# cure-lab/MagicDrive

Measured on NVIDIA B200. Metric: 6-view 224x400 denoising-steps/sec, higher is better.
Workload: dtype bf16

## Files before the change

magicdrive_b200/csrc/attention_tc.cuh:

```cuda
#pragma once
#include "ptx.cuh"

namespace mdb {

constexpr int ATT_BM = 128;
constexpr int ATT_BN = 128;

constexpr int ATT_MAX_SRC = 3;
struct AttnKvMaps {
  CUtensorMap k[ATT_MAX_SRC], v[ATT_MAX_SRC];
};

struct AttnTcParams {
  __nv_bfloat16* out;
  int ldo;
  int lq, lk;
  const int* kv_index;
  int n_sets;
  int n_src;
  float scale_log2;
  int q_step;
  long long* trace;
};

template <int D>
struct AttnTcCfg {
  static constexpr int KD = (D + 63) / 64;
  static constexpr int D16 = (D + 15) / 16 * 16;
  static constexpr int STAGES = (D <= 80) ? 2 : 1;
  static constexpr int TILE = ATT_BM * 128;
  static constexpr int SMEM_Q = KD * TILE;
  static constexpr int SMEM_KV = STAGES * 2 * KD * TILE;
  static constexpr int kSmemBytes = SMEM_Q + SMEM_KV + 1024 + 128 + 2 * 2 * ATT_BM * 4 ;
  static constexpr int S_COL = 0;
  static constexpr int P_COL = ATT_BN;
  static constexpr int O_COL = ATT_BN + 64;
  static constexpr int kTmemCols = (ATT_BN + 64 + D16 <= 256) ? 256 : 512;
  static constexpr int HW = D16 / 2;
  static constexpr int kThreads = 64 + 8 * 32;
};

__device__ __forceinline__ void umma_bf16_ts(uint32_t tmem_d, uint32_t tmem_a, uint64_t bdesc, uint32_t idesc,
                                             uint32_t accumulate) {
  asm volatile(
      "{\n\t"
      ".reg .pred p;\n\t"
      "setp.ne.b32 p, %4, 0;\n\t"
      "tcgen05.mma.cta_group::1.kind::f16 [%0], [%1], %2, %3, p;\n\t"
      "}\n" ::"r"(tmem_d),
      "r"(tmem_a), "l"(bdesc), "r"(idesc), "r"(accumulate)
      : "memory");
}

__device__ __forceinline__ void tmem_st_32x16(uint32_t taddr, const uint32_t (&v)[16]) {
  asm volatile(
      "tcgen05.st.sync.aligned.32x32b.x16.b32 [%0], "
      "{%1, %2, %3, %4, %5, %6, %7, %8, %9, %10, %11, %12, %13, %14, %15, %16};" ::"r"(taddr),
      "r"(v[0]), "r"(v[1]), "r"(v[2]), "r"(v[3]), "r"(v[4]), "r"(v[5]), "r"(v[6]), "r"(v[7]), "r"(v[8]), "r"(v[9]),
      "r"(v[10]), "r"(v[11]), "r"(v[12]), "r"(v[13]), "r"(v[14]), "r"(v[15])
      : "memory");
}
__device__ __forceinline__ void tmem_st_32x8(uint32_t taddr, const uint32_t (&v)[8]) {
  asm volatile("tcgen05.st.sync.aligned.32x32b.x8.b32 [%0], {%1, %2, %3, %4, %5, %6, %7, %8};" ::"r"(taddr), "r"(v[0]),
               "r"(v[1]), "r"(v[2]), "r"(v[3]), "r"(v[4]), "r"(v[5]), "r"(v[6]), "r"(v[7])
               : "memory");
}
__device__ __forceinline__ void tmem_st_wait() { asm volatile("tcgen05.wait::st.sync.aligned;" ::: "memory"); }

__device__ __forceinline__ uint64_t make_sw128_mnmajor_desc(uint32_t smem_addr_bytes, uint32_t lbo_bytes) {
  uint64_t d = 0;
  d |= static_cast<uint64_t>((smem_addr_bytes >> 4) & 0x3FFF);
  d |= static_cast<uint64_t>((lbo_bytes >> 4) & 0x3FFF) << 16;
  d |= static_cast<uint64_t>((1024u >> 4) & 0x3FFF) << 32;
  d |= static_cast<uint64_t>(1) << 46;
  d |= static_cast<uint64_t>(2) << 61;
  return d;
}

template <int D>
__global__ void __launch_bounds__(AttnTcCfg<D>::kThreads, (D <= 64) ? 2 : 1)
attention_tc_kernel(const __grid_constant__ CUtensorMap tmQ, const __grid_constant__ AttnKvMaps kvm,
                    const AttnTcParams p) {
  using Cfg = AttnTcCfg<D>;
  constexpr int KD = Cfg::KD, D16 = Cfg::D16, STAGES = Cfg::STAGES, TILE = Cfg::TILE;
  extern __shared__ uint8_t smem_raw[];
  uint8_t* smem = reinterpret_cast<uint8_t*>((reinterpret_cast<uintptr_t>(smem_raw) + 1023) & ~uintptr_t(1023));
  uint8_t* smQ = smem;
  uint8_t* smK = smQ + Cfg::SMEM_Q;
  uint8_t* smV = smK + STAGES * KD * TILE;
  uint64_t* bars = reinterpret_cast<uint64_t*>(smV + STAGES * KD * TILE);
  uint64_t* q_full = bars;
  uint64_t* kv_full = bars + 1;
  uint64_t* kv_empty = bars + 3;
  uint64_t* s_full = bars + 5;
  uint64_t* p_full = bars + 6;
  uint64_t* o_full = bars + 7;
  uint64_t* o_free = bars + 8;
  uint32_t* tmem_slot = reinterpret_cast<uint32_t*>(bars + 9);
  float* xchg = reinterpret_cast<float*>(bars + 16);

  const int warp = threadIdx.x >> 5, lane = threadIdx.x & 31;
  const int b = blockIdx.z, head = blockIdx.y, q0 = blockIdx.x * ATT_BM;
  const int ntiles = (p.lk + ATT_BN - 1) / ATT_BN;
  const int total_iters = ntiles * p.n_sets;

  if (warp == 0 && lane == 0) {
    prefetch_tmap(&tmQ);
    for (int i = 0; i < p.n_src; ++i) {
      prefetch_tmap(&kvm.k[i]);
      prefetch_tmap(&kvm.v[i]);
    }
  }
  if (warp == 1 && lane == 0) {
    mbar_init(q_full, 1);
    for (int i = 0; i < 2; ++i) {
      mbar_init(&kv_full[i], 1);
      mbar_init(&kv_empty[i], 1);
    }
    mbar_init(s_full, 1);
    mbar_init(p_full, 8);
    mbar_init(o_full, 1);
    mbar_init(o_free, 8);
    fence_barrier_init();
  }
  if (warp == 2) {
    tmem_alloc(tmem_slot, Cfg::kTmemCols);
    tmem_relinquish();
  }
  tc_fence_before();
  __syncthreads();
  tc_fence_after();
  const uint32_t tmem_base = *tmem_slot;
  asm volatile("griddepcontrol.wait;" ::: "memory");
  asm volatile("griddepcontrol.launch_dependents;" ::: "memory");

  if (warp == 0) {
    if (elect_one()) {
      mbar_arrive_expect_tx(q_full, KD * TILE);
#pragma unroll
      for (int c = 0; c < KD; ++c) tma_load_4d(&tmQ, q_full, smQ + c * TILE, c * 64, head, q0, b);
      int stage = 0;
      uint32_t phase = 0;
      for (int set = 0; set < p.n_sets; ++set) {
        const int kve = p.kv_index ? p.kv_index[b * p.n_sets + set] : b;
        const int kvb = kve & 0xffffff;
        const CUtensorMap* km = &kvm.k[kve >> 24];
        const CUtensorMap* vm = &kvm.v[kve >> 24];
        for (int j = 0; j < ntiles; ++j) {
          mbar_wait(&kv_empty[stage], phase ^ 1);
          mbar_arrive_expect_tx(&kv_full[stage], 2 * KD * TILE);
#pragma unroll
          for (int c = 0; c < KD; ++c) {
            tma_load_4d(km, &kv_full[stage], smK + (stage * KD + c) * TILE, c * 64, head, j * ATT_BN, kvb);
            tma_load_4d(vm, &kv_full[stage], smV + (stage * KD + c) * TILE, c * 64, head, j * ATT_BN, kvb);
          }
          if (++stage == STAGES) {
            stage = 0;
            phase ^= 1;
          }
        }
      }
    }
  } else if (warp == 1) {
    constexpr uint32_t idesc_s = make_idesc_bf16(ATT_BM, ATT_BN);
    constexpr uint32_t idesc_o = make_idesc_bf16(ATT_BM, D16) | (1u << 16);
    const uint32_t tmem_s = tmem_base + Cfg::S_COL;
    const uint32_t tmem_o = tmem_base + Cfg::O_COL;
    mbar_wait(q_full, 0);
    int stage = 0;
    uint32_t phase = 0;
    auto issue_s = [&](int st) {
      if (elect_one()) {
#pragma unroll
        for (int k = 0; k < D16 / 16; ++k) {
          const int c = k / 4, kk = k % 4;
          const uint64_t adesc = make_sw128_kmajor_desc(smem_u32(smQ + c * TILE)) + 2 * kk;
          const uint64_t bdesc = make_sw128_kmajor_desc(smem_u32(smK + (st * KD + c) * TILE)) + 2 * kk;
          umma_bf16(tmem_s, adesc, bdesc, idesc_s, k > 0 ? 1u : 0u);
        }
        umma_commit(s_full);
      }
      __syncwarp();
    };
    mbar_wait(&kv_full[0], 0);
    tc_fence_after();
    issue_s(0);
    for (int it = 0; it < total_iters; ++it) {
      mbar_wait(p_full, it & 1);
      mbar_wait(o_free, (it & 1) ^ 1);
      tc_fence_after();
      if (elect_one()) {
#pragma unroll
        for (int k = 0; k < ATT_BN / 16; ++k) {
          const uint64_t bdesc = make_sw128_mnmajor_desc(smem_u32(smV + stage * KD * TILE), TILE) + (2048u >> 4) * k;
          umma_bf16_ts(tmem_o, tmem_base + Cfg::P_COL + 8 * k, bdesc, idesc_o, k > 0 ? 1u : 0u);
        }
        umma_commit(o_full);
        umma_commit(&kv_empty[stage]);
      }
      __syncwarp();
      if (++stage == STAGES) {
        stage = 0;
        phase ^= 1;
      }
      if (it + 1 < total_iters) {
        mbar_wait(&kv_full[stage], phase);
        tc_fence_after();
        issue_s(stage);
      }
    }
  } else {
    constexpr int HW = Cfg::HW;
    const int q = warp & 3;
    const int hlf = (warp - 2) >> 2;
    const int row = q * 32 + lane;
    const uint32_t lane_base = tmem_base + (static_cast<uint32_t>(q * 32) << 16);
    const uint32_t tmem_s = lane_base + Cfg::S_COL + hlf * 64;
    const uint32_t tmem_p = lane_base + Cfg::P_COL + hlf * 32;
    const uint32_t tmem_o = lane_base + Cfg::O_COL + hlf * HW;
    const int qrow = q0 + row;
    __nv_bfloat16* orow = p.out + (static_cast<long long>(b) * p.lq + qrow) * p.ldo + head * D + hlf * HW;
    constexpr int NVALID = (D - HW >= HW) ? HW : (D - HW);
    const int nvalid = hlf ? NVALID : HW;
    const float sc = p.scale_log2;
    int it = 0;
    for (int set = 0; set < p.n_sets; ++set) {
      float o[HW];
#pragma unroll
      for (int i = 0; i < HW; ++i) o[i] = 0.f;
      float m = -INFINITY, l = 0.f;
      for (int j = 0; j < ntiles; ++j, ++it) {
        mbar_wait(s_full, it & 1);
        tc_fence_after();
        const int kbase = j * ATT_BN + hlf * 64;
        const bool tail = (kbase + 64 > p.lk);
        float mx = -INFINITY;
#pragma unroll 1
        for (int c = 0; c < 64; c += 32) {
          uint32_t v[32];
          tmem_ld_32x32(tmem_s + c, v);
          tmem_ld_wait();
          if (!tail) {
#pragma unroll
            for (int i = 0; i < 32; ++i) mx = fmaxf(mx, __uint_as_float(v[i]));
          } else {
#pragma unroll
            for (int i = 0; i < 32; ++i)
              if (kbase + c + i < p.lk) mx = fmaxf(mx, __uint_as_float(v[i]));
          }
        }
        float* xb = xchg + (it & 1) * 256;
        xb[hlf * 128 + row] = mx;
        asm volatile("bar.sync %0, 64;" ::"r"(1 + q) : "memory");
        mx = fmaxf(mx, xb[(hlf ^ 1) * 128 + row]);
        const float m_new = fmaxf(m, mx * sc);
        const float corr = exp2f(m - m_new);
        m = m_new;
        float rs = 0.f;
#pragma unroll 1
        for (int c = 0; c < 64; c += 32) {
          uint32_t v[32];
          tmem_ld_32x32(tmem_s + c, v);
          tmem_ld_wait();
          uint32_t pk[16];
          if (!tail) {
#pragma unroll
            for (int i = 0; i < 32; i += 2) {
              const float p0 = exp2f(fmaf(__uint_as_float(v[i]), sc, -m_new));
              const float p1 = exp2f(fmaf(__uint_as_float(v[i + 1]), sc, -m_new));
              rs += p0 + p1;
              pk[i >> 1] = pack_bf16(p0, p1);
            }
          } else {
#pragma unroll
            for (int i = 0; i < 32; i += 2) {
              const float p0 = (kbase + c + i < p.lk) ? exp2f(fmaf(__uint_as_float(v[i]), sc, -m_new)) : 0.f;
              const float p1 = (kbase + c + i + 1 < p.lk) ? exp2f(fmaf(__uint_as_float(v[i + 1]), sc, -m_new)) : 0.f;
              rs += p0 + p1;
              pk[i >> 1] = pack_bf16(p0, p1);
            }
          }
          tmem_st_32x16(tmem_p + (c >> 1), pk);
        }
        tmem_st_wait();
        l = l * corr + rs;
        tc_fence_before();
        __syncwarp();
        if (lane == 0) mbar_arrive(p_full);
        mbar_wait(o_full, it & 1);
        tc_fence_after();
#pragma unroll
        for (int c = 0; c < HW; c += 8) {
          uint32_t v[8];
          tmem_ld_32x8(tmem_o + c, v);
          tmem_ld_wait();
#pragma unroll
          for (int i = 0; i < 8; ++i) o[c + i] = o[c + i] * corr + __uint_as_float(v[i]);
        }
        tc_fence_before();
        __syncwarp();
        if (lane == 0) mbar_arrive(o_free);
      }
      float* xb = xchg + (it & 1) * 256;
      asm volatile("bar.sync %0, 64;" ::"r"(1 + q) : "memory");
      xb[hlf * 128 + row] = l;
      asm volatile("bar.sync %0, 64;" ::"r"(1 + q) : "memory");
      const float inv = 1.0f / (l + xb[(hlf ^ 1) * 128 + row]);
      asm volatile("bar.sync %0, 64;" ::"r"(1 + q) : "memory");
      if (qrow < p.lq) {
#pragma unroll
        for (int c = 0; c < HW; c += 8) {
          if (c >= nvalid) break;
          float f[8];
#pragma unroll
          for (int i = 0; i < 8; ++i) f[i] = o[c + i] * inv;
          if (set > 0) {
            const uint4 prev = *reinterpret_cast<const uint4*>(orow + c);
            const __nv_bfloat162* ph = reinterpret_cast<const __nv_bfloat162*>(&prev);
#pragma unroll
            for (int i = 0; i < 4; ++i) {
              const float2 pf = __bfloat1622float2(ph[i]);
              f[2 * i] = __bfloat162float(__float2bfloat16_rn(f[2 * i])) + pf.x;
              f[2 * i + 1] = __bfloat162float(__float2bfloat16_rn(f[2 * i + 1])) + pf.y;
            }
          }
          *reinterpret_cast<uint4*>(orow + c) =
              make_uint4(pack_bf16(f[0], f[1]), pack_bf16(f[2], f[3]), pack_bf16(f[4], f[5]), pack_bf16(f[6], f[7]));
        }
      }
    }
  }

  __syncthreads();
  if (warp == 2) {
    tc_fence_after();
    tmem_dealloc(tmem_base, Cfg::kTmemCols);
  }
}

}
```

magicdrive_b200/csrc/capi_attention.cu:

```cuda
#include <cuda_bf16.h>
#include <cuda_runtime.h>

#include <stdlib.h>

#include "../../include/magicdrive_b200.h"
#define MDB_NEED_TENSORMAP
#include "common_host.h"
#include <string.h>
#include "attention_tc.cuh"
#include "attention_tc2.cuh"

static long long* g_attn_trace = nullptr;

namespace {

bool make_qkv_map(CUtensorMap* m, const void* ptr, int d, int heads, int l, int b, int ld) {
  mdb::EncodeTiledFn enc = mdb::get_encode();
  if (!enc) return false;
  cuuint64_t dims[4] = {(cuuint64_t)d, (cuuint64_t)heads, (cuuint64_t)l, (cuuint64_t)b};
  cuuint64_t strides[3] = {(cuuint64_t)d * 2, (cuuint64_t)ld * 2, (cuuint64_t)l * ld * 2};
  cuuint32_t box[4] = {64u, 1u, (cuuint32_t)mdb::ATT_BM, 1u};
  cuuint32_t estr[4] = {1u, 1u, 1u, 1u};
  return enc(m, CU_TENSOR_MAP_DATA_TYPE_BFLOAT16, 4, const_cast<void*>(ptr), dims, strides, box, estr,
             CU_TENSOR_MAP_INTERLEAVE_NONE, CU_TENSOR_MAP_SWIZZLE_128B, CU_TENSOR_MAP_L2_PROMOTION_L2_256B,
             CU_TENSOR_MAP_FLOAT_OOB_FILL_NONE) == CUDA_SUCCESS;
}

struct KvSources {
  const void* k[mdb::ATT_MAX_SRC];
  const void* v[mdb::ATT_MAX_SRC];
  int ldk[mdb::ATT_MAX_SRC], ldv[mdb::ATT_MAX_SRC], b_kv[mdb::ATT_MAX_SRC];
  int n;
};

bool make_kv_maps(mdb::AttnKvMaps* m, const KvSources& s, int d, int heads, int lk) {
  for (int i = 0; i < mdb::ATT_MAX_SRC; ++i) {
    const int j = i < s.n ? i : 0;
    if (!make_qkv_map(&m->k[i], s.k[j], d, heads, lk, s.b_kv[j], s.ldk[j]) ||
        !make_qkv_map(&m->v[i], s.v[j], d, heads, lk, s.b_kv[j], s.ldv[j]))
      return false;
  }
  return true;
}

int attn_num_sms() {
  static int sms = 0;
  if (!sms) {
    int dev = 0;
    cudaGetDevice(&dev);
    if (cudaDeviceGetAttribute(&sms, cudaDevAttrMultiProcessorCount, dev) != cudaSuccess || sms <= 0) sms = 148;
  }
  return sms;
}

int multi_q_step(int b, int heads, int lq, int lk, int n_sets) {
  if (lk > mdb::ATT_BN || n_sets != 1) return 0;
  const char* e = getenv("MDB_ATTN_MULTIQ");
  if (e && e[0] == '0') return 0;
  const int nq = (lq + mdb::ATT_BM - 1) / mdb::ATT_BM;
  const long long per_tile_ctas = static_cast<long long>(b) * heads;
  const long long slots = 2LL * attn_num_sms();
  if (per_tile_ctas * nq <= slots) return 0;
  long long gx = slots / per_tile_ctas;
  if (gx < 1) gx = 1;
  if (gx >= nq) return 0;
  return static_cast<int>(gx);
}

template <typename Cfg, typename Kernel>
int launch_tc(Kernel kernel, const char* name, const void* q, int ldq, const KvSources& src, void* out, int ldo, int b, int heads,
              int lq, int lk, int d, const int* kv_index, int n_sets, float scale, cudaStream_t st, bool* attr, bool allow_multi_q = false) {
  if (!*attr) {
    cudaError_t e = cudaFuncSetAttribute(kernel, cudaFuncAttributeMaxDynamicSharedMemorySize, Cfg::kSmemBytes);
    if (e != cudaSuccess) return mdb::set_error(MDB_ERR_CUDA, "%s smem attr: %s", name, cudaGetErrorString(e));
    *attr = true;
  }
  CUtensorMap tq;
  mdb::AttnKvMaps kvm;
  if (!make_qkv_map(&tq, q, d, heads, lq, b, ldq) || !make_kv_maps(&kvm, src, d, heads, lk))
    return mdb::set_error(MDB_ERR_CUDA, "mdb_attention: cuTensorMapEncodeTiled failed (d=%d heads=%d lq=%d lk=%d)", d, heads, lq, lk);
  mdb::AttnTcParams p;
  p.out = static_cast<__nv_bfloat16*>(out);
  p.ldo = ldo, p.lq = lq, p.lk = lk, p.kv_index = kv_index, p.n_sets = n_sets, p.n_src = src.n;
  p.scale_log2 = scale * 1.4426950408889634f;
  p.trace = g_attn_trace;
  p.q_step = allow_multi_q ? multi_q_step(b, heads, lq, lk, n_sets) : 0;
  dim3 grid(p.q_step > 0 ? p.q_step : (lq + mdb::ATT_BM - 1) / mdb::ATT_BM, heads, b);
  cudaError_t le = mdb::launch_pdl(kernel, grid, dim3(Cfg::kThreads), Cfg::kSmemBytes, st, tq, kvm, p);
  if (le != cudaSuccess) return mdb::set_error(MDB_ERR_CUDA, "%s launch: %s", name, cudaGetErrorString(le));
  cudaError_t e2 = cudaGetLastError();
  if (e2 != cudaSuccess) return mdb::set_error(MDB_ERR_CUDA, "%s: %s", name, cudaGetErrorString(e2));
  return MDB_OK;
}

template <int D>
int launch_attention_tc(const void* q, int ldq, const KvSources& src, void* out, int ldo, int b, int heads, int lq, int lk,
                        const int* kv_index, int n_sets, float scale, cudaStream_t st) {
  static bool attr = false;
  return launch_tc<mdb::AttnTcCfg<D>>(mdb::attention_tc_kernel<D>, "attention_tc_kernel", q, ldq, src, out, ldo, b, heads, lq, lk, D,
                                      kv_index, n_sets, scale, st, &attr);
}

template <int D, bool DOUBLE_S>
int launch_attention_tc2(const void* q, int ldq, const KvSources& src, void* out, int ldo, int b, int heads, int lq, int lk,
                         const int* kv_index, int n_sets, float scale, cudaStream_t st) {
  if constexpr (!DOUBLE_S) {
    if (multi_q_step(b, heads, lq, lk, n_sets) > 0) {
      static bool attr_mq = false;
      return launch_tc<mdb::AttnTc2Cfg<D, false>>(mdb::attention_tc2_kernel<D, false, true>, "attention_tc2_kernel<multi-Q>", q, ldq, src,
                                                  out, ldo, b, heads, lq, lk, D, kv_index, n_sets, scale, st, &attr_mq, true);
    }
  }
  static bool attr = false;
  return launch_tc<mdb::AttnTc2Cfg<D, DOUBLE_S>>(mdb::attention_tc2_kernel<D, DOUBLE_S, false>, "attention_tc2_kernel", q, ldq, src, out,
                                                 ldo, b, heads, lq, lk, D, kv_index, n_sets, scale, st, &attr, false);
}

enum class AttnKernel { kTc, kTc2, kTc2Double };
AttnKernel attention_kernel_choice() {
  const char* e = getenv("MDB_ATTN_KERNEL");
  if (e && !strcmp(e, "tc2d")) return AttnKernel::kTc2Double;
  if (e && !strcmp(e, "tc")) return AttnKernel::kTc;
  return AttnKernel::kTc2;
}

int attention_dispatch(const void* q, int ldq, const KvSources& src, void* out, int ldo, int b, int heads, int lq, int lk, int d,
                       const int* kv_index, int n_sets, float scale, cudaStream_t st) {
  using namespace mdb;
  const AttnKernel which = attention_kernel_choice();
#define MDB_TC2(DD, DBL) return launch_attention_tc2<DD, DBL>(q, ldq, src, out, ldo, b, heads, lq, lk, kv_index, n_sets, scale, st)
  if (which != AttnKernel::kTc) {
    const bool dbl = which == AttnKernel::kTc2Double;
    switch (d) {
      case 40: if (dbl) MDB_TC2(40, true); else MDB_TC2(40, false);
      case 32: if (dbl) MDB_TC2(32, true); else MDB_TC2(32, false);
      case 64: if (dbl) MDB_TC2(64, true); else MDB_TC2(64, false);
      case 80: MDB_TC2(80, true);
      default: break;
    }
  }
#undef MDB_TC2
  switch (d) {
    case 40: return launch_attention_tc<40>(q, ldq, src, out, ldo, b, heads, lq, lk, kv_index, n_sets, scale, st);
    case 80: return launch_attention_tc<80>(q, ldq, src, out, ldo, b, heads, lq, lk, kv_index, n_sets, scale, st);
    case 160: return launch_attention_tc<160>(q, ldq, src, out, ldo, b, heads, lq, lk, kv_index, n_sets, scale, st);
    case 32: return launch_attention_tc<32>(q, ldq, src, out, ldo, b, heads, lq, lk, kv_index, n_sets, scale, st);
    case 64: return launch_attention_tc<64>(q, ldq, src, out, ldo, b, heads, lq, lk, kv_index, n_sets, scale, st);
    default: return set_error(MDB_ERR_UNSUPPORTED, "mdb_attention: head dim %d not instantiated (32, 40, 64, 80, 160)", d);
  }
}

}

extern "C" int mdb_attention_multi(const void* q, int ldq, int n_src, const void* const* k, const int* ldk, const void* const* v,
                                   const int* ldv, const int* b_kv, void* out, int ldo, int b, int heads, int lq, int lk, int d,
                                   const int* kv_index, int n_sets, float scale, void* stream) {
  using namespace mdb;
  if (!q || !k || !v || !ldk || !ldv || !b_kv || !out) return set_error(MDB_ERR_INVALID, "mdb_attention: null pointer");
  if (n_src < 1 || n_src > ATT_MAX_SRC) return set_error(MDB_ERR_INVALID, "mdb_attention: 1..%d K/V sources", ATT_MAX_SRC);
  if (n_sets < 1 || n_sets > 2 || (n_sets == 2 && !kv_index))
    return set_error(MDB_ERR_INVALID, "mdb_attention: n_sets must be 1 or 2 (2 needs kv_index)");
  if (scale <= 0.f) return set_error(MDB_ERR_INVALID, "mdb_attention: scale must be positive");
  if (lq <= 0 || lk <= 0 || b <= 0 || heads <= 0) return set_error(MDB_ERR_INVALID, "mdb_attention: bad shape");
  if (ldq % 8 || ldo % 8) return set_error(MDB_ERR_UNSUPPORTED, "mdb_attention: strides must be multiples of 8");
  KvSources src;
  src.n = n_src;
  for (int i = 0; i < n_src; ++i) {
    if (!k[i] || !v[i] || b_kv[i] <= 0) return set_error(MDB_ERR_INVALID, "mdb_attention: bad K/V source %d", i);
    if (ldk[i] % 8 || ldv[i] % 8) return set_error(MDB_ERR_UNSUPPORTED, "mdb_attention: strides must be multiples of 8");
    src.k[i] = k[i], src.v[i] = v[i], src.ldk[i] = ldk[i], src.ldv[i] = ldv[i], src.b_kv[i] = b_kv[i];
  }
  if (!kv_index && (n_src != 1 || b_kv[0] != b)) return set_error(MDB_ERR_INVALID, "mdb_attention: b_kv != b or several sources need kv_index");
  return attention_dispatch(q, ldq, src, out, ldo, b, heads, lq, lk, d, kv_index, n_sets, scale, static_cast<cudaStream_t>(stream));
}

extern "C" int mdb_attention(const void* q, int ldq, const void* k, int ldk, const void* v, int ldv, void* out, int ldo, int b,
                             int b_kv, int heads, int lq, int lk, int d, const int* kv_index, int n_sets, float scale,
                             void* stream) {
  return mdb_attention_multi(q, ldq, 1, &k, &ldk, &v, &ldv, &b_kv, out, ldo, b, heads, lq, lk, d, kv_index, n_sets, scale, stream);
}

extern "C" int mdb_attention_debug_trace(void* device_i64_384) {
  g_attn_trace = static_cast<long long*>(device_i64_384);
  return MDB_OK;
}
```

Measured before the change: 122.7.

## Add persistent ping-pong attention kernel processing two Q tiles per CTA

Adds a persistent attention kernel in which each CTA owns pairs of 128-row Q tiles. Two softmax warpgroups alternate, so the tensor-core QK/PV work for one tile overlaps the softmax of the other, and a 4-stage K/V TMA pipeline is shared between them. The kernel becomes the default for long Q sequences with head dim 32/40/64 and more than one K tile. The aim is to hide softmax latency and remove per-tile launch and setup cost, in exchange for a complex barrier protocol, full TMEM use and heavy shared-memory use that limit occupancy to one CTA per SM.

```diff
diff --git a/magicdrive_b200/csrc/attention_pp.cuh b/magicdrive_b200/csrc/attention_pp.cuh
--- /dev/null
+++ b/magicdrive_b200/csrc/attention_pp.cuh
@@ -0,0 +1,436 @@
+#pragma once
+#include "attention_tc2.cuh"
+
+namespace mdb {
+
+template <int D>
+struct AttnPpCfg {
+  static constexpr int KD = (D + 63) / 64;
+  static constexpr int D16 = (D + 15) / 16 * 16;
+  static constexpr int TILE = ATT_BM * 128;
+  static constexpr int STAGES = 4;
+  static constexpr int SMEM_Q = 2 * 2 * KD * TILE;
+  static constexpr int SMEM_KV = STAGES * 2 * KD * TILE;
+  static constexpr int kSmemBytes = SMEM_Q + SMEM_KV + 1024  + 256  + 2 * 2 * 2 * ATT_BM * 4 ;
+  static constexpr int kTmemCols = 512;
+  static constexpr int HW = D16 / 2;
+  static constexpr int kThreads = 64 + 16 * 32;
+  __host__ __device__ static constexpr int o_col(int t, int half) { return 256 + t * 128 + half * 64; }
+  static_assert(KD == 1 && D16 <= 64, "two O accumulators per tile at 64-column spacing");
+  static_assert(kSmemBytes <= 227 * 1024, "shared memory");
+};
+
+constexpr int ATT_PP_BAR_AB = 9, ATT_PP_BAR_BA = 10;
+
+template <int D>
+__global__ void __launch_bounds__(AttnPpCfg<D>::kThreads, 1)
+attention_pp_kernel(const __grid_constant__ CUtensorMap tmQ, const __grid_constant__ AttnKvMaps kvm, const AttnTcParams p) {
+  using Cfg = AttnPpCfg<D>;
+  constexpr int KD = Cfg::KD, D16 = Cfg::D16, STAGES = Cfg::STAGES, TILE = Cfg::TILE, HW = Cfg::HW;
+  extern __shared__ uint8_t smem_raw[];
+  uint8_t* smem = reinterpret_cast<uint8_t*>((reinterpret_cast<uintptr_t>(smem_raw) + 1023) & ~uintptr_t(1023));
+  uint8_t* smQ = smem;
+  uint8_t* smK = smQ + Cfg::SMEM_Q;
+  uint8_t* smV = smK + STAGES * KD * TILE;
+  uint64_t* bars = reinterpret_cast<uint64_t*>(smV + STAGES * KD * TILE);
+  uint64_t* q_full = bars;
+  uint64_t* q_empty = bars + 2;
+  uint64_t* kv_full = bars + 4;
+  uint64_t* kv_empty = bars + 8;
+  uint64_t* s_full = bars + 12;
+  uint64_t* p_full = bars + 14;
+  uint64_t* pv_done = bars + 16;
+  uint64_t* o_full = bars + 18;
+  uint64_t* o_free = bars + 20;
+  uint32_t* tmem_slot = reinterpret_cast<uint32_t*>(bars + 22);
+  float* xm = reinterpret_cast<float*>(bars + 32);
+  float* xl = xm + 4 * ATT_BM;
+
+  const int warp = threadIdx.x >> 5, lane = threadIdx.x & 31;
+  const int ntiles = (p.lk + ATT_BN - 1) / ATT_BN;
+  const int nq = (p.lq + ATT_BM - 1) / ATT_BM;
+  const int npairs = (nq + 1) / 2;
+  const int n_items = p.batch * p.heads * npairs;
+  const int my_items = (n_items - static_cast<int>(blockIdx.x) + static_cast<int>(gridDim.x) - 1) / static_cast<int>(gridDim.x);
+  const int T = ntiles * p.n_sets;
+  const int G = my_items * T;
+  struct Item {
+    int b, head, q0;
+    bool live_b;
+  };
+  auto item_of = [&](int n) {
+    const int item = static_cast<int>(blockIdx.x) + n * static_cast<int>(gridDim.x);
+    const int pair = item % npairs, bh = item / npairs;
+    return Item{bh / p.heads, bh % p.heads, pair * 2 * ATT_BM, 2 * pair + 1 < nq};
+  };
+  long long* const trace = (p.trace != nullptr && blockIdx.x == 0) ? p.trace : nullptr;
+#define MDB_ATRACE(slot, g_, k)                                                        \
+  do {                                                                                 \
+    if (trace && lane == 0 && (g_) < 16) trace[((slot) * 16 + (g_)) * 8 + (k)] = clock64(); \
+  } while (0)
+
+  if (warp == 0 && lane == 0) {
+    prefetch_tmap(&tmQ);
+    for (int i = 0; i < p.n_src; ++i) {
+      prefetch_tmap(&kvm.k[i]);
+      prefetch_tmap(&kvm.v[i]);
+    }
+  }
+  if (warp == 1 && lane == 0) {
+    for (int i = 0; i < 2; ++i) {
+      mbar_init(&q_full[i], 1);
+      mbar_init(&q_empty[i], 1);
+      mbar_init(&s_full[i], 1);
+      mbar_init(&p_full[i], 8);
+      mbar_init(&pv_done[i], 1);
+      mbar_init(&o_full[i], 1);
+      mbar_init(&o_free[i], 8);
+    }
+    for (int i = 0; i < STAGES; ++i) {
+      mbar_init(&kv_full[i], 1);
+      mbar_init(&kv_empty[i], 1);
+    }
+    fence_barrier_init();
+  }
+  if (warp == 2) {
+    tmem_alloc(tmem_slot, Cfg::kTmemCols);
+    tmem_relinquish();
+  }
+  tc_fence_before();
+  __syncthreads();
+  tc_fence_after();
+  const uint32_t tmem_base = *tmem_slot;
+  asm volatile("griddepcontrol.wait;" ::: "memory");
+  asm volatile("griddepcontrol.launch_dependents;" ::: "memory");
+
+  if (warp == 0) {
+    if (elect_one()) {
+      int stage = 0;
+      uint32_t phase = 0;
+      for (int n = 0; n < my_items; ++n) {
+        const Item it = item_of(n);
+        const int qb = n & 1;
+        if (n >= 2) mbar_wait(&q_empty[qb], static_cast<uint32_t>((n >> 1) - 1) & 1u);
+        mbar_arrive_expect_tx(&q_full[qb], (it.live_b ? 2 : 1) * KD * TILE);
+#pragma unroll
+        for (int c = 0; c < KD; ++c) {
+          tma_load_4d(&tmQ, &q_full[qb], smQ + ((qb * 2 + 0) * KD + c) * TILE, c * 64, it.head, it.q0, it.b);
+          if (it.live_b) tma_load_4d(&tmQ, &q_full[qb], smQ + ((qb * 2 + 1) * KD + c) * TILE, c * 64, it.head, it.q0 + ATT_BM, it.b);
+        }
+        for (int set = 0; set < p.n_sets; ++set) {
+          const int kve = p.kv_index ? p.kv_index[it.b * p.n_sets + set] : it.b;
+          const int kvb = kve & 0xffffff;
+          const CUtensorMap* km = &kvm.k[kve >> 24];
+          const CUtensorMap* vm = &kvm.v[kve >> 24];
+          for (int j = 0; j < ntiles; ++j) {
+            mbar_wait(&kv_empty[stage], phase ^ 1);
+            mbar_arrive_expect_tx(&kv_full[stage], 2 * KD * TILE);
+#pragma unroll
+            for (int c = 0; c < KD; ++c) {
+              tma_load_4d(km, &kv_full[stage], smK + (stage * KD + c) * TILE, c * 64, it.head, j * ATT_BN, kvb);
+              tma_load_4d(vm, &kv_full[stage], smV + (stage * KD + c) * TILE, c * 64, it.head, j * ATT_BN, kvb);
+            }
+            if (++stage == STAGES) {
+              stage = 0;
+              phase ^= 1;
+            }
+          }
+        }
+      }
+    }
+  } else if (warp == 1) {
+    constexpr uint32_t idesc_s = make_idesc_bf16(ATT_BM, ATT_BN);
+    constexpr uint32_t idesc_o = make_idesc_bf16(ATT_BM, D16) | (1u << 16);
+    struct Cur {
+      int n, set, j, r;
+      bool live_b;
+    };
+    auto advance = [&](Cur c) {
+      ++c.r;
+      if (++c.j == ntiles) {
+        c.j = 0;
+        ++c.set;
+      }
+      if (c.r == T) {
+        c.r = c.j = c.set = 0;
+        ++c.n;
+        c.live_b = c.n < my_items && item_of(c.n).live_b;
+      }
+      return c;
+    };
+    auto issue_qk = [&](int t, int g, const Cur& c) {
+      const int st = g % STAGES;
+      if (t == 0) {
+        if (c.r == 0) mbar_wait(&q_full[c.n & 1], static_cast<uint32_t>(c.n >> 1) & 1u);
+        mbar_wait(&kv_full[st], static_cast<uint32_t>(g / STAGES) & 1u);
+        tc_fence_after();
+      }
+      if (elect_one()) {
+        if (t == 0 || c.live_b) {
+          const uint32_t tmem_s = tmem_base + static_cast<uint32_t>(t * ATT_BN);
+          const uint8_t* q = smQ + ((c.n & 1) * 2 + t) * KD * TILE;
+#pragma unroll
+          for (int k = 0; k < D16 / 16; ++k) {
+            const int cc = k / 4, kk = k % 4;
+            const uint64_t adesc = make_sw128_kmajor_desc(smem_u32(q + cc * TILE)) + 2 * kk;
+            const uint64_t bdesc = make_sw128_kmajor_desc(smem_u32(smK + (st * KD + cc) * TILE)) + 2 * kk;
+            umma_bf16(tmem_s, adesc, bdesc, idesc_s, k > 0 ? 1u : 0u);
+          }
+          umma_commit(&s_full[t]);
+        } else {
+          mbar_arrive(&s_full[t]);
+        }
+        if (t == 1 && c.r == T - 1) umma_commit(&q_empty[c.n & 1]);
+      }
+      __syncwarp();
+    };
+    Cur cur{0, 0, 0, 0, my_items > 0 && item_of(0).live_b};
+    Cur nxt = advance(cur);
+    if (G > 0) {
+      issue_qk(0, 0, cur);
+      issue_qk(1, 0, cur);
+    }
+    for (int g = 0; g < G; ++g) {
+      const int st = g % STAGES, j = cur.j;
+      const int os = cur.n * p.n_sets + cur.set;
+#pragma unroll
+      for (int t = 0; t < 2; ++t) {
+        if (t == 0) MDB_ATRACE(0, g, 0);
+        mbar_wait(&p_full[t], static_cast<uint32_t>(g) & 1u);
+        MDB_ATRACE(0, g, 1 + t);
+        if (j == 0 && os > 0) mbar_wait(&o_free[t], static_cast<uint32_t>(os - 1) & 1u);
+        tc_fence_after();
+        if (elect_one()) {
+          if (t == 0 || cur.live_b) {
+#pragma unroll
+            for (int k = 0; k < ATT_BN / 16; ++k) {
+              const int half = k >> 2;
+              const uint32_t tmem_a = tmem_base + static_cast<uint32_t>(t * ATT_BN + half * 64 + 8 * (k & 3));
+              const uint32_t tmem_d = tmem_base + static_cast<uint32_t>(Cfg::o_col(t, half));
+              const uint64_t bdesc = make_sw128_mnmajor_desc(smem_u32(smV + st * KD * TILE), TILE) + (2048u >> 4) * k;
+              umma_bf16_ts(tmem_d, tmem_a, bdesc, idesc_o, (j > 0 || (k & 3) > 0) ? 1u : 0u);
+            }
+          }
+          umma_commit(&pv_done[t]);
+          if (t == 1) umma_commit(&kv_empty[st]);
+          if (j == ntiles - 1) umma_commit(&o_full[t]);
+        }
+        __syncwarp();
+        if (g + 1 < G) issue_qk(t, g + 1, nxt);
+      }
+      MDB_ATRACE(0, g, 3);
+      cur = nxt;
+      nxt = advance(nxt);
+    }
+  } else {
+    const int grp = (warp - 2) >> 3;
+    const int q = warp & 3;
+    const int hlf = ((warp - 2) >> 2) & 1;
+    const int row = q * 32 + lane;
+    const uint32_t lane_base = tmem_base + (static_cast<uint32_t>(q * 32) << 16);
+    const uint32_t tmem_acc = lane_base + Cfg::o_col(grp, hlf);
+    constexpr int NVALID = (D - HW >= HW) ? HW : (D - HW);
+    const int nvalid = hlf ? NVALID : HW;
+    const float sc = p.scale_log2;
+    const int tslot = (warp == 2) ? 1 : ((warp == 10) ? 2 : -1);
+    float* const my_xm = xm + grp * 2 * ATT_BM;
+    float* const my_xl = xl + grp * 2 * ATT_BM;
+    int g = 0;
+    for (int n = 0; n < my_items; ++n) {
+      const Item itm = item_of(n);
+      const bool live = grp == 0 || itm.live_b;
+      const int qrow = itm.q0 + grp * ATT_BM + row;
+      __nv_bfloat16* orow = p.out + (static_cast<long long>(itm.b) * p.lq + qrow) * p.ldo + itm.head * D + hlf * HW;
+      for (int set = 0; set < p.n_sets; ++set) {
+        float m_ref = -INFINITY, l = 0.f;
+        for (int j = 0; j < ntiles; ++j, ++g) {
+          const uint32_t tmem_s = lane_base + static_cast<uint32_t>(grp * ATT_BN + hlf * 64);
+          if (tslot > 0) MDB_ATRACE(tslot, g, 0);
+          mbar_wait(&s_full[grp], static_cast<uint32_t>(g) & 1u);
+          tc_fence_after();
+          if (tslot > 0) MDB_ATRACE(tslot, g, 1);
+#ifdef MDB_ATTN_PP_TOKEN
+          if (grp == 0) {
+            if (g > 0) asm volatile("bar.sync %0, 512;" ::"n"(ATT_PP_BAR_BA) : "memory");
+          } else {
+            asm volatile("bar.sync %0, 512;" ::"n"(ATT_PP_BAR_AB) : "memory");
+          }
+          if (tslot > 0) MDB_ATRACE(tslot, g, 7);
+#endif
+          float rs = 0.f;
+          uint32_t pk[32];
+          if (live) {
+          const int nval = p.lk - (j * ATT_BN + hlf * 64);
+          const bool tail = nval < 64;
+          bool done = false;
+#ifndef MDB_ATTN_NO_PIPELINED_SOFTMAX
+          if (!tail && j > 0) {
+            uint32_t a[16], b[16];
+            tmem_ld_32x16(tmem_s, a);
+            tmem_ld_wait();
+            bool ok = true;
+#pragma unroll
+            for (int c = 0; c < 4; ++c) {
+              uint32_t(&cur)[16] = (c & 1) ? b : a;
+              uint32_t(&nxt)[16] = (c & 1) ? a : b;
+              if (c < 3) tmem_ld_32x16(tmem_s + 16 * (c + 1), nxt);
+              float m4[4] = {-INFINITY, -INFINITY, -INFINITY, -INFINITY};
+#pragma unroll
+              for (int i = 0; i < 16; ++i) m4[i & 3] = fmaxf(m4[i & 3], __uint_as_float(cur[i]));
+              const float cm = fmaxf(fmaxf(m4[0], m4[1]), fmaxf(m4[2], m4[3])) * sc;
+              ok = ok && !(cm > m_ref + ATT_LAZY_LOG2);
+#pragma unroll
+              for (int i = 0; i < 16; i += 2) {
+                const float p0 = exp2f(fmaf(__uint_as_float(cur[i]), sc, -m_ref));
+                const float p1 = exp2f(fmaf(__uint_as_float(cur[i + 1]), sc, -m_ref));
+                rs += p0 + p1;
+                pk[8 * c + (i >> 1)] = pack_bf16(p0, p1);
+              }
+              if (c < 3) tmem_ld_wait();
+            }
+            done = !__any_sync(0xffffffffu, !ok);
+            if (tslot > 0) MDB_ATRACE(tslot, g, 2);
+            if (tslot > 0) MDB_ATRACE(tslot, g, 3);
+          }
+#endif
+          if (!done) {
+          rs = 0.f;
+          uint32_t v0[32], v1[32];
+          tmem_ld_32x32(tmem_s, v0);
+          tmem_ld_32x32(tmem_s + 32, v1);
+          tmem_ld_wait();
+          if (tslot > 0) MDB_ATRACE(tslot, g, 2);
+          float mx = -INFINITY;
+          if (!tail) {
+            float m4[4] = {-INFINITY, -INFINITY, -INFINITY, -INFINITY};
+#pragma unroll
+            for (int i = 0; i < 32; ++i) m4[i & 3] = fmaxf(m4[i & 3], fmaxf(__uint_as_float(v0[i]), __uint_as_float(v1[i])));
+            mx = fmaxf(fmaxf(m4[0], m4[1]), fmaxf(m4[2], m4[3]));
+          } else {
+#pragma unroll
+            for (int i = 0; i < 32; ++i) {
+              if (i < nval) mx = fmaxf(mx, __uint_as_float(v0[i]));
+              if (32 + i < nval) mx = fmaxf(mx, __uint_as_float(v1[i]));
+            }
+          }
+          if (tslot > 0) MDB_ATRACE(tslot, g, 3);
+          const float m_new = mx * sc;
+          const bool need = m_new > m_ref + ATT_LAZY_LOG2;
+          if (__any_sync(0xffffffffu, need)) {
+            if (j > 0) {
+              mbar_wait(&pv_done[grp], static_cast<uint32_t>(g - 1) & 1u);
+              tc_fence_after();
+              const float corr = need ? exp2f(m_ref - m_new) : 1.0f;
+#pragma unroll 1
+              for (int c = 0; c < D16; c += 8) {
+                uint32_t o[8];
+                tmem_ld_32x8(tmem_acc + c, o);
+                tmem_ld_wait();
+#pragma unroll
+                for (int i = 0; i < 8; ++i) o[i] = __float_as_uint(__uint_as_float(o[i]) * corr);
+                tmem_st_32x8(tmem_acc + c, o);
+              }
+              l *= corr;
+            }
+            if (need) m_ref = m_new;
+          }
+          if (!tail) {
+#pragma unroll
+            for (int i = 0; i < 32; i += 2) {
+              const float p0 = exp2f(fmaf(__uint_as_float(v0[i]), sc, -m_ref));
+              const float p1 = exp2f(fmaf(__uint_as_float(v0[i + 1]), sc, -m_ref));
+              const float p2 = exp2f(fmaf(__uint_as_float(v1[i]), sc, -m_ref));
+              const float p3 = exp2f(fmaf(__uint_as_float(v1[i + 1]), sc, -m_ref));
+              rs += (p0 + p1) + (p2 + p3);
+              pk[i >> 1] = pack_bf16(p0, p1);
+              pk[16 + (i >> 1)] = pack_bf16(p2, p3);
+            }
+          } else {
+#pragma unroll
+            for (int i = 0; i < 32; i += 2) {
+              const float p0 = (i < nval) ? exp2f(fmaf(__uint_as_float(v0[i]), sc, -m_ref)) : 0.f;
+              const float p1 = (i + 1 < nval) ? exp2f(fmaf(__uint_as_float(v0[i + 1]), sc, -m_ref)) : 0.f;
+              const float p2 = (32 + i < nval) ? exp2f(fmaf(__uint_as_float(v1[i]), sc, -m_ref)) : 0.f;
+              const float p3 = (33 + i < nval) ? exp2f(fmaf(__uint_as_float(v1[i + 1]), sc, -m_ref)) : 0.f;
+              rs += (p0 + p1) + (p2 + p3);
+              pk[i >> 1] = pack_bf16(p0, p1);
+              pk[16 + (i >> 1)] = pack_bf16(p2, p3);
+            }
+          }
+          }
+          }
+          if (tslot > 0) MDB_ATRACE(tslot, g, 4);
+#ifdef MDB_ATTN_PP_TOKEN
+          if (grp == 0) {
+            asm volatile("bar.arrive %0, 512;" ::"n"(ATT_PP_BAR_AB) : "memory");
+          } else {
+            if (g + 1 < G) asm volatile("bar.arrive %0, 512;" ::"n"(ATT_PP_BAR_BA) : "memory");
+          }
+#endif
+          if (live) {
+            tmem_st_32x16(tmem_s, *reinterpret_cast<const uint32_t(*)[16]>(&pk[0]));
+            tmem_st_32x16(tmem_s + 16, *reinterpret_cast<const uint32_t(*)[16]>(&pk[16]));
+            tmem_st_wait();
+          }
+          if (tslot > 0) MDB_ATRACE(tslot, g, 5);
+          l += rs;
+          tc_fence_before();
+          __syncwarp();
+          if (lane == 0) mbar_arrive(&p_full[grp]);
+          if (tslot > 0) MDB_ATRACE(tslot, g, 6);
+        }
+        mbar_wait(&o_full[grp], static_cast<uint32_t>(n * p.n_sets + set) & 1u);
+        tc_fence_after();
+        if (live) {
+          my_xm[hlf * ATT_BM + row] = m_ref;
+          my_xl[hlf * ATT_BM + row] = l;
+          asm volatile("bar.sync %0, 64;" ::"r"(1 + q + 4 * grp) : "memory");
+          const float m_other = my_xm[(hlf ^ 1) * ATT_BM + row], l_other = my_xl[(hlf ^ 1) * ATT_BM + row];
+          asm volatile("bar.sync %0, 64;" ::"r"(1 + q + 4 * grp) : "memory");
+          const float m_tot = fmaxf(m_ref, m_other);
+          const float w_me = exp2f(m_ref - m_tot), w_other = exp2f(m_other - m_tot);
+          const float inv = 1.0f / (l * w_me + l_other * w_other);
+          const float wa = (hlf ? w_other : w_me) * inv, wb = (hlf ? w_me : w_other) * inv;
+          const uint32_t tmem_oa = lane_base + Cfg::o_col(grp, 0) + hlf * HW, tmem_ob = lane_base + Cfg::o_col(grp, 1) + hlf * HW;
+#pragma unroll
+          for (int c = 0; c < HW; c += 8) {
+            if (c >= nvalid) break;
+            uint32_t oa[8], ob[8];
+            tmem_ld_32x8(tmem_oa + c, oa);
+            tmem_ld_32x8(tmem_ob + c, ob);
+            tmem_ld_wait();
+            if (qrow < p.lq) {
+              float f[8];
+#pragma unroll
+              for (int i = 0; i < 8; ++i) f[i] = __uint_as_float(oa[i]) * wa + __uint_as_float(ob[i]) * wb;
+              if (set > 0) {
+                const uint4 prev = *reinterpret_cast<const uint4*>(orow + c);
+                const __nv_bfloat162* ph = reinterpret_cast<const __nv_bfloat162*>(&prev);
+#pragma unroll
+                for (int i = 0; i < 4; ++i) {
+                  const float2 pf = __bfloat1622float2(ph[i]);
+                  f[2 * i] = __bfloat162float(__float2bfloat16_rn(f[2 * i])) + pf.x;
+                  f[2 * i + 1] = __bfloat162float(__float2bfloat16_rn(f[2 * i + 1])) + pf.y;
+                }
+              }
+              *reinterpret_cast<uint4*>(orow + c) =
+                  make_uint4(pack_bf16(f[0], f[1]), pack_bf16(f[2], f[3]), pack_bf16(f[4], f[5]), pack_bf16(f[6], f[7]));
+            }
+          }
+        }
+        tc_fence_before();
+        __syncwarp();
+        if (lane == 0) mbar_arrive(&o_free[grp]);
+      }
+    }
+  }
+
+#undef MDB_ATRACE
+  __syncthreads();
+  if (warp == 2) {
+    tc_fence_after();
+    tmem_dealloc(tmem_base, Cfg::kTmemCols);
+  }
+}
+
+}
diff --git a/magicdrive_b200/csrc/attention_tc.cuh b/magicdrive_b200/csrc/attention_tc.cuh
--- a/magicdrive_b200/csrc/attention_tc.cuh
+++ b/magicdrive_b200/csrc/attention_tc.cuh
@@ -21,6 +21,7 @@
   float scale_log2;
   int q_step;
   long long* trace;
+  int batch, heads;
 };
 
 template <int D>
diff --git a/magicdrive_b200/csrc/capi_attention.cu b/magicdrive_b200/csrc/capi_attention.cu
--- a/magicdrive_b200/csrc/capi_attention.cu
+++ b/magicdrive_b200/csrc/capi_attention.cu
@@ -9,6 +9,7 @@
 #include <string.h>
 #include "attention_tc.cuh"
 #include "attention_tc2.cuh"
+#include "attention_pp.cuh"
 
 static long long* g_attn_trace = nullptr;
 
@@ -69,7 +70,8 @@
 
 template <typename Cfg, typename Kernel>
 int launch_tc(Kernel kernel, const char* name, const void* q, int ldq, const KvSources& src, void* out, int ldo, int b, int heads,
-              int lq, int lk, int d, const int* kv_index, int n_sets, float scale, cudaStream_t st, bool* attr, bool allow_multi_q = false) {
+              int lq, int lk, int d, const int* kv_index, int n_sets, float scale, cudaStream_t st, bool* attr, bool allow_multi_q = false,
+              bool persistent_pairs = false) {
   if (!*attr) {
     cudaError_t e = cudaFuncSetAttribute(kernel, cudaFuncAttributeMaxDynamicSharedMemorySize, Cfg::kSmemBytes);
     if (e != cudaSuccess) return mdb::set_error(MDB_ERR_CUDA, "%s smem attr: %s", name, cudaGetErrorString(e));
@@ -85,7 +87,12 @@
   p.scale_log2 = scale * 1.4426950408889634f;
   p.trace = g_attn_trace;
   p.q_step = allow_multi_q ? multi_q_step(b, heads, lq, lk, n_sets) : 0;
+  p.batch = b, p.heads = heads;
   dim3 grid(p.q_step > 0 ? p.q_step : (lq + mdb::ATT_BM - 1) / mdb::ATT_BM, heads, b);
+  if (persistent_pairs) {
+    const long long items = static_cast<long long>(b) * heads * (((lq + mdb::ATT_BM - 1) / mdb::ATT_BM + 1) / 2);
+    grid = dim3(static_cast<unsigned>(items < attn_num_sms() ? items : attn_num_sms()), 1, 1);
+  }
   cudaError_t le = mdb::launch_pdl(kernel, grid, dim3(Cfg::kThreads), Cfg::kSmemBytes, st, tq, kvm, p);
   if (le != cudaSuccess) return mdb::set_error(MDB_ERR_CUDA, "%s launch: %s", name, cudaGetErrorString(le));
   cudaError_t e2 = cudaGetLastError();
@@ -116,18 +123,38 @@
                                                  ldo, b, heads, lq, lk, D, kv_index, n_sets, scale, st, &attr, false);
 }
 
-enum class AttnKernel { kTc, kTc2, kTc2Double };
+template <int D>
+int launch_attention_pp(const void* q, int ldq, const KvSources& src, void* out, int ldo, int b, int heads, int lq, int lk,
+                        const int* kv_index, int n_sets, float scale, cudaStream_t st) {
+  static bool attr = false;
+  return launch_tc<mdb::AttnPpCfg<D>>(mdb::attention_pp_kernel<D>, "attention_pp_kernel", q, ldq, src, out, ldo, b, heads, lq, lk, D,
+                                      kv_index, n_sets, scale, st, &attr, false, true);
+}
+
+constexpr int ATT_PP_MIN_QTILES = 32;
+enum class AttnKernel { kDefault, kTc, kTc2, kTc2Double, kPp };
 AttnKernel attention_kernel_choice() {
   const char* e = getenv("MDB_ATTN_KERNEL");
+  if (e && !strcmp(e, "pp")) return AttnKernel::kPp;
+  if (e && !strcmp(e, "tc2")) return AttnKernel::kTc2;
   if (e && !strcmp(e, "tc2d")) return AttnKernel::kTc2Double;
   if (e && !strcmp(e, "tc")) return AttnKernel::kTc;
-  return AttnKernel::kTc2;
+  return AttnKernel::kDefault;
 }
 
 int attention_dispatch(const void* q, int ldq, const KvSources& src, void* out, int ldo, int b, int heads, int lq, int lk, int d,
                        const int* kv_index, int n_sets, float scale, cudaStream_t st) {
   using namespace mdb;
   const AttnKernel which = attention_kernel_choice();
+  const bool long_q = (lq + ATT_BM - 1) / ATT_BM >= ATT_PP_MIN_QTILES;
+  if ((which == AttnKernel::kPp || (which == AttnKernel::kDefault && long_q)) && lk > ATT_BN) {
+    switch (d) {
+      case 40: return launch_attention_pp<40>(q, ldq, src, out, ldo, b, heads, lq, lk, kv_index, n_sets, scale, st);
+      case 32: return launch_attention_pp<32>(q, ldq, src, out, ldo, b, heads, lq, lk, kv_index, n_sets, scale, st);
+      case 64: return launch_attention_pp<64>(q, ldq, src, out, ldo, b, heads, lq, lk, kv_index, n_sets, scale, st);
+      default: break;
+    }
+  }
 #define MDB_TC2(DD, DBL) return launch_attention_tc2<DD, DBL>(q, ldq, src, out, ldo, b, heads, lq, lk, kv_index, n_sets, scale, st)
   if (which != AttnKernel::kTc) {
     const bool dbl = which == AttnKernel::kTc2Double;
```

Result: no change. 122.7, median of 6 (-0.0%).
